# subhk/FeastKit.jl

Measured on AMD Instinct MI355X. Metric: eigenpairs/sec + max residual, 16-node contour, higher is better.
Workload: dtype f64

## Files before the change

### feastkit.jl_amd/csrc/fh_api.hip

```cpp
#include "fh_common.hpp"
#include "fh_kernels.hpp"
#include "fh_dense.hpp"
#include "fh_banded.hpp"
#include "fh_eig.hpp"
#include "fh_comm.hpp"
#include "../../include/feasthip.h"

#include <algorithm>
#include <chrono>
#include <thread>
#include <cmath>
#include <cstring>

int fh_get_buf(feasthip_ctx* h, const char* name, size_t bytes, void** out) {
    auto it = h->bufs.find(name);
    if (it != h->bufs.end() && it->second.second >= bytes) {
        *out = it->second.first;
        return 0;
    }
    if (it != h->bufs.end()) {
        hipStreamSynchronize(h->stream);
        hipFree(it->second.first);
        h->bufs.erase(it);
    }
// ... 372 lines not shown
    for (int e = 0; e < count; ++e) h->node_ids[e] = first + e;
    return 0;
}

extern "C" int feasthip_set_node_list(feasthip_handle h, int count, const int* indices) {
    if (!h) return FEASTHIP_ERROR_INTERNAL;
    if (count < 0 || (count > 0 && !indices)) { h->last_error = "feasthip_set_node_list: bad arguments"; return FEASTHIP_ERROR_FPM; }
    for (int e = 0; e < count; ++e)
        if (indices[e] < 0 || indices[e] >= (int)h->zne.size()) {
            h->last_error = "feasthip_set_node_list: index outside the contour";
            return FEASTHIP_ERROR_FPM;
        }
    h->node_ids.assign(indices, indices + count);
    h->node_first = count > 0 ? indices[0] : 0;
    h->node_count = count;
    return 0;
}

extern "C" int feasthip_set_column_mask(feasthip_handle h, int64_t m, const int* mask) {
    if (!h) return FEASTHIP_ERROR_INTERNAL;
    if (m < 0 || m > (1 << 20)) { h->last_error = "set_column_mask: m out of range"; return FEASTHIP_ERROR_M0; }
    h->col_mask.clear();
    if (mask && m > 0) h->col_mask.assign(mask, mask + m);
    return 0;
}

extern "C" int feasthip_set_solver(feasthip_handle h, int kind, double rtol, double atol, int maxit, int restart,
                                   int factor_precision, int cache_factors) {
    if (!h) return FEASTHIP_ERROR_INTERNAL;
    if (kind < 0 || kind > 4 || rtol < 0 || atol < 0 || maxit <= 0 || restart < 0 ||
        (factor_precision != 64 && factor_precision != 32)) {
        h->last_error = "feasthip_set_solver: invalid option";
        return FEASTHIP_ERROR_FPM;
    }
    h->solver = kind; h->rtol = rtol; h->atol = atol; h->maxit = maxit; h->restart = restart;
    h->factor_precision = factor_precision; h->cache_factors = cache_factors;
    return 0;
}


struct fh_op_call {
    const void* X; size_t x_stride;
    void* Y; size_t y_stride;
    const cplx* coefA; const cplx* coefB;
    const void* Bvec; size_t b_stride;
    const void* U; size_t u_stride;
    int dot_mode; cplx* partial1; cplx* partial2;
    const int* node_active;
    int nodes;
    int m = FH_MAX_LD;
    int uniform_coef = 0;
    int prec = 64;
    const cplx* colscale = nullptr;
};

static bool fh_row_kernel_ok(feasthip_ctx* h, int ld) {
    static const bool row_off = getenv("FH_SPMM_ROW") && atoi(getenv("FH_SPMM_ROW")) == 0;
    return h->kind == 2 && ld == 64 && !h->csr.is_complex && h->csr.rp8 && !row_off;
}

static int fh_apply_operator(feasthip_ctx* h, int ld, const fh_op_call& c) {
    if (h->kind == 2) {
        fh_spmm_args a;
        a.rowptr = h->csr.rowptr; a.col = h->csr.col; a.aval = h->csr.aval; a.bval = h->csr.bval;
        a.N = (int)h->csr.N; a.nodes = c.nodes;
        a.X = c.X; a.x_node_stride = c.x_stride; a.Y = c.Y; a.y_node_stride = c.y_stride;
        a.coefA = c.coefA; a.coefB = c.coefB; a.Bvec = c.Bvec; a.b_node_stride = c.b_stride;
        a.U = c.U; a.u_node_stride = c.u_stride; a.dot_mode = c.dot_mode;
        a.partial1 = c.partial1; a.partial2 = c.partial2; a.node_active = c.node_active;
        a.counters = h->profiling ? h->d_counters : nullptr; a.m = c.m; a.uniform_coef = c.uniform_coef; a.prec = c.prec;
        static const bool no_lds = !(getenv("FH_LDS_SPMM") && atoi(getenv("FH_LDS_SPMM")) != 0);
        const bool lds_kernel = h->csr.lcol && c.prec == 64 && !no_lds && c.nodes <= 64 && c.dot_mode != 6;
        a.nblk_rows = h->csr.nblk; a.blk_start = h->csr.blk_start; a.ext_ptr = h->csr.ext_ptr; a.ext_idx = h->csr.ext_idx;
        a.lcol = lds_kernel ? h->csr.lcol : nullptr;
        a.use_row_kernel = (fh_row_kernel_ok(h, ld) && !lds_kernel) ? 1 : 0;
        a.colscale = c.colscale;
        if (c.colscale && (lds_kernel || c.prec != 64 || h->csr.is_complex)) { h->last_error = "internal: column-scaled operand needs a gather kernel over a real matrix on complex128 panels"; return -1; }
        a.rp8 = h->csr.rp8; a.col8 = h->csr.col8; a.a8 = h->csr.a8; a.b8 = h->csr.b8;
        fh_prof_begin(h, "spmm");
        fh_launch_spmm(a, ld, h->csr.is_complex != 0, h->csr.b_identity != 0, fh_spmm_grid(a.N, ld), h->stream);
        fh_prof_end(h);
        if (a.use_row_kernel) return fh_spmm_row_grid(a.N);
        if (lds_kernel) return (8 / (ld / 16)) * fh_spmm_lds_slots(a.nblk_rows, ld);
        return fh_spmm_partials(a.N, ld);
    }
    fh_dense_op_args a;
    a.A = h->dense.A; a.B = h->dense.B; a.N = (int)h->dense.N; a.is_complex = h->dense.is_complex;
    a.nodes = c.nodes; a.X = (const cplx*)c.X; a.x_node_stride = c.x_stride; a.Y = (cplx*)c.Y; a.y_node_stride = c.y_stride;
    a.coefA = c.coefA; a.coefB = c.coefB; a.Bvec = (const cplx*)c.Bvec; a.b_node_stride = c.b_stride;
    a.U = (const cplx*)c.U; a.u_node_stride = c.u_stride; a.dot_mode = c.dot_mode;
    a.partial1 = c.partial1; a.partial2 = c.partial2; a.node_active = c.node_active;
    int nblk = fh_dense_op_nblk(a.N);
    fh_prof_begin(h, "dense_op");
    fh_launch_dense_op(a, ld, nblk, h->stream);
    fh_prof_end(h);
    return nblk;
}

static int fh_op_nblk(feasthip_ctx* h, int ld) {
    if (h->kind == 2) return std::max(std::max(fh_spmm_partials((int)h->csr.N, ld), ld == 64 ? fh_spmm_row_grid((int)h->csr.N) : 0),
                                      h->csr.lcol ? (8 / (ld / 16)) * fh_spmm_lds_slots(h->csr.nblk, ld) : 0);
    return fh_dense_op_nblk((int)h->dense.N);
}
static const int* fh_perm(feasthip_ctx* h) { return h->kind == 2 ? h->csr.perm : nullptr; }
static int64_t fh_N(feasthip_ctx* h) { return h->kind == 2 ? h->csr.N : h->dense.N; }
static bool fh_b_identity(feasthip_ctx* h) { return h->kind == 2 ? h->csr.b_identity != 0 : h->dense.b_identity != 0; }

static int fh_check_problem(feasthip_ctx* h, int64_t m, int wide = 0) {
    if (!h) return FEASTHIP_ERROR_INTERNAL;
    if (h->poisoned) { h->last_error = "handle poisoned by an earlier device failure: destroy it"; return FEASTHIP_ERROR_INTERNAL; }
    if (h->kind == 0) { h->last_error = "no matrix set (feasthip_set_dense / feasthip_set_csr)"; return FEASTHIP_ERROR_N; }
    if (m <= 0 || (!wide && m > FH_MAX_LD) || m > fh_N(h)) {
        h->last_error = wide ? "block width m must satisfy 1 <= m <= N" : "block width m must satisfy 1 <= m <= min(N, 64)";
        return FEASTHIP_ERROR_M0;
    }
    return 0;
}

static int fh_upload_coefs(feasthip_ctx* h, const char* name, const std::vector<cplx>& host, cplx** dev) {
    void* p = nullptr;
    int rc = fh_get_buf(h, name, host.size() * sizeof(cplx), &p);
    if (rc) return rc;
    const size_t bytes = host.size() * sizeof(cplx);
    if (h->pin && bytes <= h->pin_cap / 4) {
        const size_t need = (bytes + 63) & ~(size_t)63;
        if (h->pin_off + need > h->pin_cap) {
            FH_CHECK(hipStreamSynchronize(h->stream));
            h->pin_off = 0;
        }
        memcpy(h->pin + h->pin_off, host.data(), bytes);
// ... 118 lines not shown
    fa.atol_scale = nullptr; fa.mode = method; fa.col_mask = nullptr;
    if (h->mask_live && !h->col_mask.empty()) {
        std::vector<int> mk(ld, 1);
        for (int c = 0; c < ld && c < (int)h->col_mask.size(); ++c) mk[c] = h->col_mask[c];
        if ((rc = fh_get_buf(h, "kry_colmask", ld * sizeof(int), &p))) return rc;
        FH_CHECK(hipMemcpyAsync(p, mk.data(), ld * sizeof(int), hipMemcpyHostToDevice, h->stream));
        FH_CHECK(hipStreamSynchronize(h->stream));
        fa.col_mask = (const int*)p;
    }
    fh_vec_args va;
    memset(&va, 0, sizeof(va));
    va.N = N; va.node_stride = panel; va.R = R; va.Rhat = Rh; va.P = P; va.V = V; va.S = S; va.T = T;
    va.s = s; va.partial1 = part1; va.partial2 = part2; va.prec = prec;
    va.counters = h->profiling ? h->d_counters : nullptr;
    va.sum_acc = sum_acc; va.wnode = d_wnode; va.sum_scale = (sum_acc && prec == 32) ? r0_64 : nullptr; va.nodes = nodes;

    void* Xk = X;
    const bool shared_start = shared_src && sum_acc && method == 1 && prec == 64;
    if (shared_start) {
    } else if (prec == 64) {
        oc.prec = 64; oc.X = X; oc.x_stride = panel; oc.Y = R; oc.y_stride = panel; oc.Bvec = RHS; oc.b_stride = 0;
        oc.dot_mode = 3; oc.node_active = nullptr;
        fa.nblk = fh_apply_operator(h, ld, oc);
        res.op_calls += 1;
    } else {
        void* q;
        if ((rc = fh_get_buf(h, "kry_r64", (size_t)nodes * panel * sizeof(cplx), &q))) return rc;
        cplx* R64 = (cplx*)q;
        oc.prec = 64; oc.X = X; oc.x_stride = panel; oc.Y = R64; oc.y_stride = panel; oc.Bvec = RHS; oc.b_stride = 0;
        oc.dot_mode = 3; oc.node_active = nullptr;
        int nb = fh_apply_operator(h, ld, oc);
        res.op_calls += 1;
        fh_fin_args f0 = fa;
        f0.nblk = nb; f0.rtol = 0.0; f0.atol = 0.0; f0.mode = 0;
        fh_launch_fin_init(f0, ld, nodes, h->stream);
        FH_CHECK(hipMemcpyAsync(r0_64, s.r0norm, nl * sizeof(double), hipMemcpyDeviceToDevice, h->stream));
        cplxf* D = (cplxf*)vec(6);
        cplxf* RHS32 = (cplxf*)vec(7);
        fh_launch_narrow_scaled(R64, panel, RHS32, panel, r0_64, N, ld, nblk_vec, nodes, h->stream);
        FH_CHECK(hipMemsetAsync(D, 0, (size_t)nodes * panel * sizeof(cplxf), h->stream));
        FH_CHECK(hipMemcpyAsync(R, RHS32, (size_t)nodes * panel * sizeof(cplxf), hipMemcpyDeviceToDevice, h->stream));
        Xk = D;
        std::vector<double> hr0(nl), hinv(nl);
        FH_CHECK(hipMemcpyAsync(hr0.data(), r0_64, nl * sizeof(double), hipMemcpyDeviceToHost, h->stream));
        FH_CHECK(hipStreamSynchronize(h->stream));
        for (size_t i = 0; i < nl; ++i) hinv[i] = hr0[i] > 0 ? 1.0 / hr0[i] : 0.0;
        FH_CHECK(hipMemcpyAsync(inv_r0, hinv.data(), nl * sizeof(double), hipMemcpyHostToDevice, h->stream));
        FH_CHECK(hipStreamSynchronize(h->stream));
        fa.atol_scale = inv_r0;
    }
    va.X = Xk;
    const int vprec = prec;
    const bool lazy_off = getenv("FH_NO_LAZY_START") != nullptr;
    const bool lazy = shared_start && fused && h->kind == 2 && !h->csr.is_complex && !lazy_off && (!shared_lambda || shared_lambda_host) &&
                      !(getenv("FH_LDS_SPMM") && atoi(getenv("FH_LDS_SPMM")) != 0);
    cplx* dfs = nullptr;
    if (lazy) {
        std::vector<cplx> fs(nl, cmake(1, 0));
        if (shared_lambda_host)
            for (int e = 0; e < nodes; ++e)
                for (int c = 0; c < m; ++c) fs[(size_t)e * ld + c] = cdiv(cmake(1, 0), cmake(z[e].x - shared_lambda_host[c], z[e].y));
        if ((rc = fh_upload_coefs(h, "kry_fscale", fs, &dfs))) return rc;
        fh_vec_args vs = va;
        vs.Q = shared_src; vs.first_scale = dfs;
        fh_launch_cocg_init_lazy(vs, ld, nblk_vec, nodes, h->stream);
        fa.nblk = nblk_vec;
        fh_launch_fin_init(fa, ld, nodes, h->stream);
    } else if (shared_start) {
        fh_vec_args vs = va;
        vs.Q = shared_src; vs.lambda = shared_lambda; vs.znode = dznode;
        fh_launch_cocg_init_shared(vs, ld, nblk_vec, nodes, h->stream);
        fa.nblk = nblk_vec;
        fh_launch_fin_init(fa, ld, nodes, h->stream);
    } else if (method == 1) {
        fh_launch_cocg_init(va, ld, nblk_vec, nodes, h->stream);
        fa.nblk = nblk_vec;
        fh_launch_fin_init(fa, ld, nodes, h->stream);
    } else {
        if (prec == 32) {
            fh_launch_cocg_init(va, ld, nblk_vec, nodes, h->stream);
            fa.nblk = nblk_vec;
        }
        fa.mode = 0;
        fh_launch_fin_init(fa, ld, nodes, h->stream);
        fh_launch_copy_r(va, ld, nblk_vec, nodes, h->stream);
    }
    (void)vprec;

    oc.prec = prec; oc.Bvec = nullptr; oc.b_stride = 0; oc.x_stride = panel; oc.y_stride = panel;
    const int check_every = getenv("FH_CHECK_EVERY") ? std::max(1, atoi(getenv("FH_CHECK_EVERY"))) : 16;
    (void)d_count;
    *h->h_progress = 0ull;
    int it = 0;
    unsigned tag = 0;
    bool all_done = false;
    auto t_loop0 = std::chrono::steady_clock::now();
    auto progress = [&](unsigned& seen_tag, unsigned& seen_cnt) {
        unsigned long long w = *h->h_progress;
        seen_tag = (unsigned)(w >> 32); seen_cnt = (unsigned)(w & 0xffffffffull);
    };
    while (it < h->maxit && !all_done) {
        int chunk = std::min(check_every, h->maxit - it);
        for (int k = 0; k < chunk; ++k) {
            if (method == 0) {
                oc.X = P; oc.Y = V; oc.U = Rh; oc.u_stride = panel; oc.dot_mode = 1; oc.node_active = s.node_active;
                fa.nblk = fh_apply_operator(h, ld, oc);
                fh_prof_begin(h, "dot_finalize"); fh_launch_fin_alpha(fa, ld, nodes, h->stream); fh_prof_end(h);
                fh_prof_begin(h, "bicg_s"); fh_launch_s_update(va, ld, nblk_vec, nodes, h->stream); fh_prof_end(h);
                oc.X = S; oc.Y = T; oc.U = nullptr; oc.dot_mode = 2;
                fa.nblk = fh_apply_operator(h, ld, oc);
                fh_prof_begin(h, "dot_finalize"); fh_launch_fin_omega(fa, ld, nodes, h->stream); fh_prof_end(h);
                fh_prof_begin(h, "bicg_xr"); fh_launch_xr_update(va, ld, nblk_vec, nodes, h->stream); fh_prof_end(h);
                fa.nblk = nblk_vec;
                fh_prof_begin(h, "dot_finalize"); fh_launch_fin_rho(fa, ld, nodes, h->stream); fh_prof_end(h);
                fh_prof_begin(h, "bicg_p"); fh_launch_p_update(va, ld, nblk_vec, nodes, h->stream); fh_prof_end(h);
                res.op_calls += 2;
            } else if (fused) {
                const bool first_lazy = lazy && it + k == 0;
                oc.X = first_lazy ? (const void*)shared_src : P; oc.x_stride = first_lazy ? 0 : panel; oc.colscale = first_lazy ? dfs : nullptr;
                oc.Y = V; oc.U = nullptr; oc.dot_mode = 6; oc.node_active = s.node_active;
                oc.partial1 = sp[0]; oc.partial2 = sp[1];
                va.first_src = first_lazy ? shared_src : nullptr; va.first_scale = first_lazy ? dfs : nullptr;
                fh_fused_fin_args ff;
                ff.s = s; ff.sig = sp[0]; ff.kap = sp[1];
                ff.rho = part1; ff.rr = part2; ff.tickets = d_tickets; ff.final_check = 0;
                ff.predict_stop = (h->rtol >= 1e-3 && h->atol == 0.0) ? 1 : 0;
                ff.nblk_op = fh_apply_operator(h, ld, oc);
                ff.nblk_vec = (it + k == 0) ? fa.nblk : ((lazy && it + k == 1) ? fv1_blk * fv1_seg : fv_blk * fv_seg);
                fh_prof_begin(h, "dot_finalize"); fh_launch_fused_fin(ff, ld, nodes, h->stream); fh_prof_end(h);
                fh_prof_begin(h, "cocg_vec"); fh_launch_fused_vec(va, ld, h->stream); fh_prof_end(h);
                res.op_calls += 1;
            } else {
                oc.X = P; oc.Y = V; oc.U = nullptr; oc.dot_mode = 4; oc.node_active = s.node_active;
                fa.nblk = fh_apply_operator(h, ld, oc);
                fh_prof_begin(h, "dot_finalize"); fh_launch_fin_alpha(fa, ld, nodes, h->stream); fh_prof_end(h);
                fh_prof_begin(h, "cocg_xr"); fh_launch_cocg_update(va, ld, nblk_vec, nodes, h->stream); fh_prof_end(h);
                fa.nblk = nblk_vec;
                fh_prof_begin(h, "dot_finalize"); fh_launch_fin_rho(fa, ld, nodes, h->stream); fh_prof_end(h);
                fh_prof_begin(h, "cocg_p");
                if (sum_acc) fh_launch_cocg_p_sum(va, ld, nodes, h->stream);
                else fh_launch_cocg_p(va, ld, nblk_vec, nodes, h->stream);
                fh_prof_end(h);
                res.op_calls += 1;
            }
        }
        it += chunk;
        ++tag;
        fh_launch_publish_progress(s.node_active, nodes, h->d_progress, tag, h->stream);
        unsigned st = 0, sc = 0;
        for (unsigned spins = 1;; ++spins) {
            progress(st, sc);
            if (st >= 1 && sc == 0) { all_done = true; break; }
            if (tag < 3 || st + 3 > tag) break;
            std::this_thread::sleep_for(std::chrono::microseconds(100));
            if ((spins & 2047u) == 0) {
                const hipError_t q = hipStreamQuery(h->stream);
                if (q != hipSuccess && q != hipErrorNotReady) {
                    h->last_error = std::string("device queue failed while iterating: ") + hipGetErrorString(q);
                    h->poisoned = 1;
                    return FEASTHIP_ERROR_INTERNAL;
                }
                const double waited = std::chrono::duration<double>(std::chrono::steady_clock::now() - t_loop0).count();
                const double budget = 30.0 + 0.05 * (double)h->maxit * (1.0 + (double)N * nodes / 8.0e5);
                if (waited > budget) {
                    h->last_error = "device did not make progress on the Krylov iterations within the deadline (" + std::to_string((int)budget) + " s)";
                    fh_poison_unless_drained(h, 2.0);
                    return FEASTHIP_ERROR_INTERNAL;
                }
            }
        }
    }
    if (fused && it > 0) {
        fh_fused_fin_args ff;
        ff.s = s; ff.sig = ff.kap = nullptr; ff.rho = part1; ff.rr = part2; ff.tickets = d_tickets;
        ff.nblk_op = 0; ff.nblk_vec = (lazy && it == 1) ? fv1_blk * fv1_seg : fv_blk * fv_seg; ff.final_check = 1; ff.predict_stop = 0;
        fh_launch_fused_fin(ff, ld, nodes, h->stream);
    }
    FH_CHECK(hipStreamSynchronize(h->stream));
    if (getenv("FH_DEBUG_TIMING"))
        fprintf(stderr, "[fh_krylov] nodes=%d its queued=%d loop wall %.3f ms\n", nodes, it,
                1e3 * std::chrono::duration<double>(std::chrono::steady_clock::now() - t_loop0).count());
    if (prec == 32 && !sum_acc)
        fh_launch_widen_axpy(X, panel, (const cplxf*)Xk, panel, r0_64, N, ld, nblk_vec, nodes, h->stream);

    std::vector<int> iters(nl), status(nl), active(nl);
    std::vector<double> rnorm(nl), r0(nl);
    FH_CHECK(hipMemcpy(iters.data(), s.iters, nl * sizeof(int), hipMemcpyDeviceToHost));
    FH_CHECK(hipMemcpy(status.data(), s.status, nl * sizeof(int), hipMemcpyDeviceToHost));
    FH_CHECK(hipMemcpy(active.data(), s.active, nl * sizeof(int), hipMemcpyDeviceToHost));
    FH_CHECK(hipMemcpy(rnorm.data(), s.rnorm, nl * sizeof(double), hipMemcpyDeviceToHost));
    FH_CHECK(hipMemcpy(r0.data(), s.r0norm, nl * sizeof(double), hipMemcpyDeviceToHost));
    res.status.assign(nodes, 0);
    for (int e = 0; e < nodes; ++e) {
        int mx = 0, st = 0;
        for (int c = 0; c < m; ++c) {
            int i = e * ld + c;
            mx = std::max(mx, iters[i]);
            res.col_iters.push_back(iters[i]);
            if (active[i] || !std::isfinite(rnorm[i])) st = std::max(st, (int)FEASTHIP_ERROR_NO_CONVERGENCE);
            else if (status[i] == 8 && !(rnorm[i] <= h->atol + h->rtol * r0[i])) st = std::max(st, (int)FEASTHIP_ERROR_NO_CONVERGENCE);
            if (r0[i] > 0) res.max_rel_res = std::max(res.max_rel_res, rnorm[i] / r0[i]);
        }
        res.iters_sum += mx;
        res.node_iters.push_back(mx);
        res.max_iters = std::max(res.max_iters, mx);
        res.status[e] = st;
    }
    return 0;
}

static int fh_gmres(feasthip_ctx* h, int ld, int m, int nodes_all, const std::vector<cplx>& z, const cplx* RHS, cplx* X,
                    size_t stride, fh_solve_result& res) {
    const int N = (int)fh_N(h);
    const size_t panel = (size_t)N * ld;
    const int mr = std::max(h->restart, 2);
    int rc;
    void* p;
    res.status.assign(nodes_all, 0);
    const size_t per_node = (size_t)(mr + 2) * panel * sizeof(cplx);
    size_t budget = (size_t)48 << 30;
    {
        size_t free_b = 0, total_b = 0;
        if (hipMemGetInfo(&free_b, &total_b) == hipSuccess) {
            auto held = h->bufs.find("gm_V");
            const size_t avail = free_b / 2 + (held != h->bufs.end() ? held->second.second : 0);
            budget = std::min(budget, std::max(avail, per_node));
        }
    }
// ... 2030 lines not shown
```

### feastkit.jl_amd/csrc/fh_kernels.hpp

```cpp
#pragma once
#include "fh_common.hpp"

struct fh_spmm_args {
    const int* rowptr; const int* col; const void* aval; const void* bval;
    int N; int nodes;
    const void* X; size_t x_node_stride;
    void* Y; size_t y_node_stride;
    const cplx* coefA; const cplx* coefB;
    const void* Bvec; size_t b_node_stride;
    const void* U; size_t u_node_stride;
    int dot_mode;
    cplx* partial1; cplx* partial2;
    const int* node_active;
    unsigned long long* counters;
    int m;
    int uniform_coef;
    int prec;
    const int* rp8 = nullptr; const int* col8 = nullptr; const double* a8 = nullptr; const double* b8 = nullptr;
    int use_row_kernel = 0;
    const cplx* colscale = nullptr;
    int nblk_rows; const int* blk_start; const int* ext_ptr; const int* ext_idx; const unsigned short* lcol;
};
int fh_spmm_grid(int N, int ld);
int fh_spmm_partials(int N, int ld);
int fh_spmm_row_grid(int N);
int fh_spmm_lds_slots(int nblk_rows, int ld);
void fh_launch_spmm(const fh_spmm_args& a, int ld, bool is_complex, bool bident, int nblk, hipStream_t st);

struct fh_vec_args {
    int N;
    size_t node_stride;
    void *X, *R, *Rhat, *P, *V, *S, *T;
    const cplx* Q;
    const double* lambda;
    const cplx* znode;
    fh_krylov_scalars s;
    cplx* partial1; cplx* partial2;
    int prec;
    unsigned long long* counters;
    const cplx* first_src;
    const cplx* first_scale;
    cplx* sum_acc;
    const cplx* wnode;
    const double* sum_scale;
    int nodes;
};
struct fh_fin_args {
    fh_krylov_scalars s;
    const cplx* partial1; const cplx* partial2;
    int nblk; int m;
    double rtol, atol;
    const double* atol_scale;
    int mode;
    const int* col_mask;
};
void fh_launch_init_guess(const fh_vec_args& a, int ld, int nblk, int nodes, hipStream_t st);
void fh_launch_copy_r(const fh_vec_args& a, int ld, int nblk, int nodes, hipStream_t st);
void fh_launch_p_update(const fh_vec_args& a, int ld, int nblk, int nodes, hipStream_t st);
void fh_launch_s_update(const fh_vec_args& a, int ld, int nblk, int nodes, hipStream_t st);
void fh_launch_xr_update(const fh_vec_args& a, int ld, int nblk, int nodes, hipStream_t st);
void fh_launch_cocg_init(const fh_vec_args& a, int ld, int nblk, int nodes, hipStream_t st);
void fh_launch_cocg_init_shared(const fh_vec_args& a, int ld, int nblk, int nodes, hipStream_t st);
void fh_launch_cocg_init_lazy(const fh_vec_args& a, int ld, int nblk, int nodes, hipStream_t st);
void fh_launch_sum_finish(const cplx* src, const cplx* rho, const cplx* acc, cplx* out, int N, int ld, int real_part, hipStream_t st);
void fh_launch_cocg_update(const fh_vec_args& a, int ld, int nblk, int nodes, hipStream_t st);
void fh_launch_cocg_p(const fh_vec_args& a, int ld, int nblk, int nodes, hipStream_t st);
void fh_launch_cocg_p_sum(const fh_vec_args& a, int ld, int nodes, hipStream_t st);
struct fh_fused_fin_args {
    fh_krylov_scalars s;
    const cplx *sig, *kap;
    const cplx *rho, *rr;
    int nblk_op, nblk_vec;
    unsigned long long* tickets;
    int final_check;
    int predict_stop;
};
void fh_launch_fused_fin(const fh_fused_fin_args& a, int ld, int nodes, hipStream_t st);
void fh_fused_vec_geometry(int N, int ld, int half, int* nblk, int* nseg, int* per_thread);
void fh_launch_fused_vec(const fh_vec_args& a, int ld, hipStream_t st);
void fh_launch_fin_init(const fh_fin_args& a, int ld, int nodes, hipStream_t st);
void fh_launch_fin_alpha(const fh_fin_args& a, int ld, int nodes, hipStream_t st);
void fh_launch_fin_omega(const fh_fin_args& a, int ld, int nodes, hipStream_t st);
void fh_launch_fin_rho(const fh_fin_args& a, int ld, int nodes, hipStream_t st);
void fh_launch_count_active(const int* node_active, int nodes, int* out, hipStream_t st);
void fh_launch_publish_progress(const int* node_active, int nodes, unsigned long long* progress, unsigned tag, hipStream_t st);
void fh_launch_narrow_scaled(const cplx* src, size_t src_stride, cplxf* dst, size_t dst_stride, const double* r0norm,
                             int N, int ld, int nblk, int nodes, hipStream_t st);
void fh_launch_widen_axpy(cplx* X, size_t x_stride, const cplxf* D, size_t d_stride, const double* r0norm,
                          int N, int ld, int nblk, int nodes, hipStream_t st);

struct fh_gmres_args {
    int N; int mr;
    size_t panel;
    cplx* V; size_t v_node_stride;
    cplx* W;
    cplx* partial;
    cplx* npartial;
    cplx* H;
    cplx* hcur;
    cplx* cs; cplx* sn;
    cplx* g;
    cplx* y;
    double* inv;
    double* r0norm; double* target; double* rnorm;
    int* active; int* iters; int* status; int* kdim;
    int* node_active;
};
int fh_gm_nchunk(int k);
size_t fh_gm_partial_elems(int mr, int nblk, int nodes, int ld);
void fh_launch_gm_orthogonalize(const fh_gmres_args& a, int ld, int k, int nblk, int nodes, hipStream_t st);
void fh_launch_gm_start(const fh_gmres_args& a, int ld, int nblk_norm, int nodes, int first, double rtol, double atol, int m, hipStream_t st);
void fh_launch_gm_givens(const fh_gmres_args& a, int ld, int k, int nblk, int nodes, hipStream_t st);
void fh_launch_gm_scale_store(const fh_gmres_args& a, int ld, const cplx* src, size_t src_node_stride, int dst_index, int nblk, int nodes,
                              hipStream_t st);
void fh_launch_gm_finish_cycle(const fh_gmres_args& a, int ld, cplx* X, size_t x_node_stride, int kmax, int nblk, int nodes, hipStream_t st);

void fh_launch_to_panel(const cplx* src, int64_t lds, int N, int m, cplx* dst, int ld, hipStream_t st, const int* perm = nullptr);
void fh_launch_from_panel(const cplx* src, int ld, int N, int m, cplx* dst, int64_t ldd, hipStream_t st, const int* perm = nullptr);
void fh_launch_panel_cols(const cplx* src, int lds, int c0, int w, int N, cplx* dst, int ldd, hipStream_t st);
void fh_launch_pack_cols(const cplx* src, int lds, int c0, int w, int N, double* dst, int ldd, int real_only, hipStream_t st);
void fh_launch_to_panel_real(const double* src, int64_t lds, int N, int m, cplx* dst, int ld, hipStream_t st);
void fh_launch_accumulate(const cplx* X, size_t node_stride, const cplx* w, int nodes, int N, int ld, const cplx* extra,
                          cplx* dst, int real_part, hipStream_t st);
size_t fh_gram_work_elems(int ld);
void fh_launch_gram(const cplx* X, const cplx* Y, int N, int ld, int bilinear, cplx* work, cplx* G,
                    hipStream_t st);
int fh_vec_nblk(int N, int ld);
int fh_kry_nblk(int N, int ld, int nodes);
void fh_launch_dot_cols(const cplx* U, const cplx* V, int N, int ld, cplx* work, cplx* out, hipStream_t st);
void fh_launch_scale_cols(cplx* X, const cplx* s, int N, int ld, hipStream_t st);
void fh_launch_normalize_cols(cplx* X, const cplx* dots, int N, int ld, int M, hipStream_t st);
void fh_launch_small_matmul(const cplx* Q, const cplx* V, int N, int ld, cplx* Xout, hipStream_t st);
// ... 19 lines not shown
```

### feastkit.jl_amd/csrc/fh_sparse.hip

```cpp
#include "fh_common.hpp"
#include "fh_kernels.hpp"

#define FH_BLOCK 256
#define FH_FIN_BLOCK 1024

template <int LD>
__device__ __forceinline__ void fh_block_reduce_cols(cplx v, cplx* red, cplx* out) {
    const int t = threadIdx.x;
    red[t] = v;
    __syncthreads();
    if (t < LD) {
        cplx s = red[t];
#pragma unroll
        for (int k = 1; k < FH_BLOCK / LD; ++k) s = cadd(s, red[t + k * LD]);
        out[t] = s;
    }
    __syncthreads();
}

static inline int fh_spmm_slots(int N, int ld) {
    const int nt = ld / 16, slices = 8 / nt;
    int rows = (N + slices - 1) / slices;
    int S = (rows + 15) / 16;
    if (S > 128) S = 128;
// ... 178 lines not shown
                d2.x += cabs2(accd);
            } else if (a.dot_mode == 3) {
                d2.x += cabs2(accd);
            } else if (a.dot_mode == 4) {
                d1 = cadd(d1, cmul(to_d(xo), accd));
            } else if (a.dot_mode == 6) {
                d1 = cadd(d1, cmul(to_d(xo), accd));
                d2 = cadd(d2, cmul(accd, accd));
            }
        }
        if (a.dot_mode != 0) {
            if (a.dot_mode == 1 || a.dot_mode == 2 || a.dot_mode == 4 || a.dot_mode == 6) {
                red[t] = d1;
                __syncthreads();
                if (t < 16) {
                    cplx s = cmake(0, 0);
                    for (int k = 0; k < 16; ++k) s = cadd(s, red[t + 16 * k]);
                    a.partial1[pbase + t] = s;
                }
                __syncthreads();
            }
            if (a.dot_mode == 2 || a.dot_mode == 3 || a.dot_mode == 6) {
                red[t] = d2;
                __syncthreads();
                if (t < 16) {
                    cplx s = cmake(0, 0);
                    for (int k = 0; k < 16; ++k) s = cadd(s, red[t + 16 * k]);
                    a.partial2[pbase + t] = s;
                }
                __syncthreads();
            }
        }
    }
}

#ifndef FH_ROW_THREADS
#define FH_ROW_THREADS 1024
#endif
#ifndef FH_ROW_WAVES
#define FH_ROW_WAVES 4
#endif
#ifndef FH_ROW_BLOCKS_MAX
#define FH_ROW_BLOCKS_MAX 1
#endif
static inline int fh_spmm_row_groups(int N, int blocks_per_cu) {
    (void)N;
    return 32 * blocks_per_cu;
}

__device__ __forceinline__ double fh_uniform(double v) {
    return __hiloint2double(__builtin_amdgcn_readfirstlane(__double2hiint(v)), __builtin_amdgcn_readfirstlane(__double2loint(v)));
}

template <typename CT, bool BIDENT, bool UNIF>
__global__ __launch_bounds__(FH_ROW_THREADS, FH_ROW_WAVES) void k_spmm_row(fh_spmm_args a) {
    constexpr int LD = 64;
    __shared__ double red[FH_ROW_THREADS / 64][64][4];
    const int lane = threadIdx.x & 63;
    const int wave = __builtin_amdgcn_readfirstlane(threadIdx.x >> 6);
    constexpr int WPB = FH_ROW_THREADS / 64;
    const int S = gridDim.x >> 3;
    const int grp = blockIdx.x & 7, slot = blockIdx.x >> 3;
    const int slice_rows = (a.N + 7) / 8;
    const int row_lo = min(a.N, grp * slice_rows);
    const int row_hi = min(a.N, row_lo + slice_rows);
    const int band = S * WPB;
    typedef const double __attribute__((address_space(4))) * cdptr;
    typedef const int __attribute__((address_space(4))) * ciptr;
    const cdptr a8 = (cdptr)a.a8;
    const cdptr b8 = (cdptr)a.b8;
    const ciptr rp8 = (ciptr)a.rp8;
    const ciptr col8 = (ciptr)a.col8;
    const int prow = blockIdx.x, nprow = gridDim.x;

    for (int node = 0; node < a.nodes; ++node) {
        const size_t pbase = ((size_t)node * nprow + prow) * LD;
        if (a.node_active && a.node_active[node] == 0) {
            if (a.dot_mode != 0 && threadIdx.x < LD) {
                if (a.partial1) a.partial1[pbase + threadIdx.x] = cmake(0, 0);
                if (a.partial2) a.partial2[pbase + threadIdx.x] = cmake(0, 0);
            }
            continue;
        }
        if (a.counters && blockIdx.x == 0 && threadIdx.x == 0) {
            const int cols = a.node_active ? a.node_active[node] : a.m;
            const int passes = (a.dot_mode == 1 || a.Bvec) ? 3 : 2;
            atomicAdd(a.counters + 0, 1ull);
            atomicAdd(a.counters + 1, (unsigned long long)(cols * passes));
        }
        const CT* __restrict__ X = (const CT*)a.X + (size_t)node * a.x_node_stride;
        CT* __restrict__ Y = (CT*)a.Y + (size_t)node * a.y_node_stride;
        const CT* __restrict__ Bv = a.Bvec ? (const CT*)a.Bvec + (size_t)node * a.b_node_stride : nullptr;
        const CT* __restrict__ U = a.U ? (const CT*)a.U + (size_t)node * a.u_node_stride : nullptr;
        cplx ca = a.coefA[node * LD + lane];
        cplx cb = a.coefB[node * LD + lane];
        if (UNIF) { ca = cmake(fh_uniform(ca.x), fh_uniform(ca.y)); cb = cmake(fh_uniform(cb.x), fh_uniform(cb.y)); }
        const bool scaled = a.colscale != nullptr;
        const cplx fs = scaled ? a.colscale[node * LD + lane] : cmake(1, 0);
        double d1x = 0.0, d1y = 0.0, d2x = 0.0, d2y = 0.0;
        for (int i = row_lo + slot * WPB + wave; i < row_hi; i += band) {
            const int c0 = rp8[i], c1 = rp8[i + 1];
            double ux = 0.0, uy = 0.0, vx = 0.0, vy = 0.0;
            const CT xown = (X + (size_t)i * LD)[lane];
            for (int ch = c0; ch < c1; ++ch) {
                const ciptr cc = col8 + (size_t)ch * 8;
                const cdptr aa = a8 + (size_t)ch * 8;
                CT xs[8];
#pragma unroll
                for (int q = 0; q < 8; ++q) {
                    const int j = cc[q];
                    if (j != i) {
                        const CT* __restrict__ rowp = X + (size_t)j * LD;
                        xs[q] = rowp[lane];
                    } else {
                        xs[q] = xown;
                    }
                }
#pragma unroll
                for (int q = 0; q < 8; ++q) {
                    const cplx x = to_d(xs[q]);
                    const double av = aa[q];
                    ux += av * x.x; uy += av * x.y;
                    if (!BIDENT) {
                        const double bv = (b8 + (size_t)ch * 8)[q];
                        vx += bv * x.x; vy += bv * x.y;
                    }
                }
            }
            cplx u = cmake(ux, uy), v = cmake(vx, vy);
            if (BIDENT) v = to_d(xown);
            cplx accd = cadd(cmul(cb, v), cmul(ca, u));
            cplx xo = to_d(xown);
            if (scaled) { accd = cmul(fs, accd); xo = cmul(fs, xo); }
            if (Bv) accd = csub(to_d(fh_ld_nt((Bv + (size_t)i * LD) + lane)), accd);
            const CT acc = cvt<CT>(accd);
            fh_st_nt((Y + (size_t)i * LD) + lane, acc);
            accd = to_d(acc);
            if (a.dot_mode == 1) {
                const cplx t1 = cmulc(to_d(fh_ld_nt((U + (size_t)i * LD) + lane)), accd);
                d1x += t1.x; d1y += t1.y;
            } else if (a.dot_mode == 2) {
                const cplx t1 = cmulc(accd, xo);
                d1x += t1.x; d1y += t1.y; d2x += cabs2(accd);
            } else if (a.dot_mode == 3) {
                d2x += cabs2(accd);
            } else if (a.dot_mode == 4) {
                const cplx t1 = cmul(xo, accd);
                d1x += t1.x; d1y += t1.y;
            } else if (a.dot_mode == 6) {
                const cplx t1 = cmul(xo, accd), t2 = cmul(accd, accd);
                d1x += t1.x; d1y += t1.y; d2x += t2.x; d2y += t2.y;
            }
        }
        if (a.dot_mode != 0) {
            red[wave][lane][0] = d1x; red[wave][lane][1] = d1y; red[wave][lane][2] = d2x; red[wave][lane][3] = d2y;
            __syncthreads();
            if (threadIdx.x < LD) {
                double s0 = 0.0, s1 = 0.0, s2 = 0.0, s3 = 0.0;
#pragma unroll
                for (int w = 0; w < WPB; ++w) { s0 += red[w][threadIdx.x][0]; s1 += red[w][threadIdx.x][1]; s2 += red[w][threadIdx.x][2]; s3 += red[w][threadIdx.x][3]; }
                if (a.partial1) a.partial1[pbase + threadIdx.x] = cmake(s0, s1);
                if (a.partial2) a.partial2[pbase + threadIdx.x] = cmake(s2, s3);
            }
            __syncthreads();
        }
    }
}

#define FH_LDS_SLOTS (FH_SPMM_R + FH_SPMM_EXT)
#define FH_LDS_RPG (FH_SPMM_R / 16)
#define FH_SEL8(arr, s) ((s) == 0 ? arr[0] : (s) == 1 ? arr[1] : (s) == 2 ? arr[2] : (s) == 3 ? arr[3] : (s) == 4 ? arr[4] : (s) == 5 ? arr[5] : (s) == 6 ? arr[6] : arr[7])
static_assert(FH_LDS_RPG == 8, "FH_SEL8 assumes eight rows per lane group");
template <typename VT, int LD, bool BIDENT>
__global__ __launch_bounds__(FH_BLOCK, 2) void k_spmm_lds(fh_spmm_args a) {
    typedef cplx CT;
    constexpr int NT = LD / 16;
    constexpr int SLICES = 8 / NT;
    extern __shared__ cplx lds_x[];
    __shared__ cplx red[FH_BLOCK];
    __shared__ int s_list[64];
    __shared__ int s_cnt;
    const int t = threadIdx.x;
    const int lane = t & 63, wave = t >> 6;
    const int g = lane >> 4, l16 = lane & 15;
    const int S = gridDim.x >> 3;
    const int grp = blockIdx.x & 7, slot = blockIdx.x >> 3;
    const int ct = grp % NT, slice = grp / NT;
    const int per = (a.nblk_rows + SLICES - 1) / SLICES;
    const int b_lo = min(a.nblk_rows, slice * per), b_hi = min(a.nblk_rows, b_lo + per);
    const int c = ct * 16 + l16;
    const VT* __restrict__ aval = (const VT*)a.aval;
    const VT* __restrict__ bval = (const VT*)a.bval;
    const int* __restrict__ rowptr = a.rowptr;
    const int* __restrict__ colidx = a.col;
    const unsigned short* __restrict__ lcol = a.lcol;
    const int prow = slice * S + slot;
    const int nprow = SLICES * S;

    if (t == 0) {
        int n = 0;
        for (int node = 0; node < a.nodes && n < 64; ++node)
            if (!a.node_active || a.node_active[node] != 0) s_list[n++] = node;
        s_cnt = n;
    }
    if (a.dot_mode != 0 && t < 16) {
        for (int node = 0; node < a.nodes; ++node) {
            const size_t pb = ((size_t)node * nprow + prow) * LD + ct * 16;
            if (a.partial1) a.partial1[pb + t] = cmake(0, 0);
            if (a.partial2) a.partial2[pb + t] = cmake(0, 0);
        }
    }
    __syncthreads();
    const int cnt_nodes = s_cnt;
    if (a.counters && blockIdx.x == 0 && t == 0) {
        unsigned long long cols = 0;
        for (int q = 0; q < cnt_nodes; ++q) cols += (unsigned long long)(a.node_active ? a.node_active[s_list[q]] : a.m);
        atomicAdd(a.counters + 0, (unsigned long long)cnt_nodes);
// ... 164 lines not shown
        hipFuncSetAttribute((const void*)k_spmm_lds<VT, LD, true>, hipFuncAttributeMaxDynamicSharedMemorySize, (int)dyn);
        hipFuncSetAttribute((const void*)k_spmm_lds<VT, LD, false>, hipFuncAttributeMaxDynamicSharedMemorySize, (int)dyn);
        attr_done = true;
    }
    dim3 grid(8 * fh_spmm_lds_slots(a.nblk_rows, LD)), block(FH_BLOCK);
    if (bident) hipLaunchKernelGGL((k_spmm_lds<VT, LD, true>), grid, block, dyn, st, a);
    else hipLaunchKernelGGL((k_spmm_lds<VT, LD, false>), grid, block, dyn, st, a);
}

template <typename CT, typename VT, int LD>
static void launch_spmm_ld(const fh_spmm_args& a, bool bident, int nblk, hipStream_t st) {
    dim3 grid(nblk), block(FH_BLOCK);
    if constexpr (sizeof(CT) == sizeof(cplx) && sizeof(VT) == sizeof(double)) {
        if (a.colscale) {
            if (bident) hipLaunchKernelGGL((k_spmm<CT, VT, LD, true, true>), grid, block, 0, st, a);
            else hipLaunchKernelGGL((k_spmm<CT, VT, LD, false, true>), grid, block, 0, st, a);
            return;
        }
    }
    if (bident)
        hipLaunchKernelGGL((k_spmm<CT, VT, LD, true>), grid, block, 0, st, a);
    else
        hipLaunchKernelGGL((k_spmm<CT, VT, LD, false>), grid, block, 0, st, a);
}
template <typename CT>
static void launch_spmm_ct(const fh_spmm_args& a, int ld, bool is_complex, bool bident, int nblk, hipStream_t st) {
    if (is_complex) {
        if (ld == 16) launch_spmm_ld<CT, cplx, 16>(a, bident, nblk, st);
        else if (ld == 32) launch_spmm_ld<CT, cplx, 32>(a, bident, nblk, st);
        else launch_spmm_ld<CT, cplx, 64>(a, bident, nblk, st);
    } else {
        if (ld == 16) launch_spmm_ld<CT, double, 16>(a, bident, nblk, st);
        else if (ld == 32) launch_spmm_ld<CT, double, 32>(a, bident, nblk, st);
        else launch_spmm_ld<CT, double, 64>(a, bident, nblk, st);
    }
}
int fh_spmm_row_grid(int N) {
    static int per_cu = 0;
    if (!per_cu) {
        int n = 0;
        if (hipOccupancyMaxActiveBlocksPerMultiprocessor(&n, k_spmm_row<cplx, false, true>, FH_ROW_THREADS, 0) != hipSuccess || n < 1) n = 1;
        per_cu = n > FH_ROW_BLOCKS_MAX ? FH_ROW_BLOCKS_MAX : n;
    }
    int S = fh_spmm_row_groups(N, per_cu);
    const int slice_rows = (N + 7) / 8, wpb = FH_ROW_THREADS / 64;
    const int need = (slice_rows + wpb - 1) / wpb;
    if (S > need) S = need < 1 ? 1 : need;
    return 8 * S;
}

void fh_launch_spmm(const fh_spmm_args& a, int ld, bool is_complex, bool bident, int nblk, hipStream_t st) {
    if (a.use_row_kernel) {
        dim3 grid(fh_spmm_row_grid(a.N)), block(FH_ROW_THREADS);
#define FH_ROW_LAUNCH(CT_, BI_) \
        do { if (a.uniform_coef) hipLaunchKernelGGL((k_spmm_row<CT_, BI_, true>), grid, block, 0, st, a); \
             else hipLaunchKernelGGL((k_spmm_row<CT_, BI_, false>), grid, block, 0, st, a); } while (0)
        if (a.prec == 32) { if (bident) FH_ROW_LAUNCH(cplxf, true); else FH_ROW_LAUNCH(cplxf, false); }
        else { if (bident) FH_ROW_LAUNCH(cplx, true); else FH_ROW_LAUNCH(cplx, false); }
#undef FH_ROW_LAUNCH
        return;
    }
    if (a.prec == 64 && a.lcol) {
        if (is_complex) {
            if (ld == 16) launch_spmm_lds<cplx, 16>(a, bident, st);
            else if (ld == 32) launch_spmm_lds<cplx, 32>(a, bident, st);
            else launch_spmm_lds<cplx, 64>(a, bident, st);
        } else {
            if (ld == 16) launch_spmm_lds<double, 16>(a, bident, st);
            else if (ld == 32) launch_spmm_lds<double, 32>(a, bident, st);
            else launch_spmm_lds<double, 64>(a, bident, st);
        }
        return;
    }
    if (a.prec == 32) launch_spmm_ct<cplxf>(a, ld, is_complex, bident, nblk, st);
    else launch_spmm_ct<cplx>(a, ld, is_complex, bident, nblk, st);
}

template <typename CT, int LD>
__global__ __launch_bounds__(FH_BLOCK) void k_init_guess(fh_vec_args a) {
    const int node = blockIdx.y;
    const size_t total = (size_t)a.N * LD;
    const int c = threadIdx.x % LD;
    cplx* X = (cplx*)a.X + (size_t)node * a.node_stride;
    cplx f = cmake(0, 0);
    if (a.lambda) {
        cplx z = a.znode[node];
        f = cdiv(cmake(1, 0), cmake(z.x - a.lambda[c], z.y));
    }
    for (size_t e = (size_t)blockIdx.x * FH_BLOCK + threadIdx.x; e < total; e += (size_t)gridDim.x * FH_BLOCK)
        X[e] = a.lambda ? cmul(a.Q[e], f) : cmake(0, 0);
}

template <typename CT, int LD>
__global__ __launch_bounds__(FH_BLOCK) void k_copy_r(fh_vec_args a) {
    const int node = blockIdx.y;
    const size_t total = (size_t)a.N * LD;
    const CT* R = (const CT*)a.R + (size_t)node * a.node_stride;
    CT* Rh = (CT*)a.Rhat + (size_t)node * a.node_stride;
    CT* P = (CT*)a.P + (size_t)node * a.node_stride;
    for (size_t e = (size_t)blockIdx.x * FH_BLOCK + threadIdx.x; e < total; e += (size_t)gridDim.x * FH_BLOCK) {
        CT r = R[e];
        Rh[e] = r;
        P[e] = r;
    }
}

template <typename CT, int LD>
__global__ __launch_bounds__(FH_BLOCK) void k_p_update(fh_vec_args a) {
    const int node = blockIdx.y;
    if (a.s.node_active[node] == 0) return;
    const size_t total = (size_t)a.N * LD;
    const int c = threadIdx.x % LD;
    if (!a.s.active[node * LD + c]) return;
    const CT beta = cvt<CT>(a.s.beta[node * LD + c]), omega = cvt<CT>(a.s.omega[node * LD + c]);
    const CT* R = (const CT*)a.R + (size_t)node * a.node_stride;
    const CT* V = (const CT*)a.V + (size_t)node * a.node_stride;
    CT* P = (CT*)a.P + (size_t)node * a.node_stride;
    for (size_t e = (size_t)blockIdx.x * FH_BLOCK + threadIdx.x; e < total; e += (size_t)gridDim.x * FH_BLOCK) {
        CT t = csub(P[e], cmul(omega, V[e]));
        P[e] = cadd(R[e], cmul(beta, t));
    }
}

template <typename CT, int LD>
__global__ __launch_bounds__(FH_BLOCK) void k_s_update(fh_vec_args a) {
    const int node = blockIdx.y;
    if (a.s.node_active[node] == 0) return;
    const size_t total = (size_t)a.N * LD;
// ... 804 lines not shown
```

Baseline: 301.2.

## Fuse COCG vector update with recomputed SpMM to skip storing A*p

The fused COCG path normally writes the operator product V = A*P, then a separate vector kernel reads it back to update R, P and the solution sum. The new mode runs the SpMM with dots only and no store, and a new row kernel recomputes A*P per row while applying the residual, direction and accumulation updates. P and V ping-pong as the input and output direction buffers, and the kernel processes nodes in groups of up to four. This removes a full panel write and read per iteration but computes the sparse product twice, so it trades memory traffic for extra gathers and FLOPs.

Measured after the change: 293.5 (median of 2 runs). 0.974x the previous value.

```diff
diff --git a/feastkit.jl_amd/csrc/fh_api.hip b/feastkit.jl_amd/csrc/fh_api.hip
--- a/feastkit.jl_amd/csrc/fh_api.hip
+++ b/feastkit.jl_amd/csrc/fh_api.hip
@@ -448,6 +448,7 @@
     int uniform_coef = 0;
     int prec = 64;
     const cplx* colscale = nullptr;
+    int no_store = 0;
 };
 
 static bool fh_row_kernel_ok(feasthip_ctx* h, int ld) {
@@ -472,6 +473,8 @@
         a.use_row_kernel = (fh_row_kernel_ok(h, ld) && !lds_kernel) ? 1 : 0;
         a.colscale = c.colscale;
         if (c.colscale && (lds_kernel || c.prec != 64 || h->csr.is_complex)) { h->last_error = "internal: column-scaled operand needs a gather kernel over a real matrix on complex128 panels"; return -1; }
+        a.no_store = c.no_store;
+        if (c.no_store && (!a.use_row_kernel || c.prec != 64 || c.dot_mode != 6 || !c.uniform_coef || c.Bvec || c.colscale)) { h->last_error = "internal: dots-only operator product needs the row kernel, fused-COCG dots and complex128 panels"; return -1; }
         a.rp8 = h->csr.rp8; a.col8 = h->csr.col8; a.a8 = h->csr.a8; a.b8 = h->csr.b8;
         fh_prof_begin(h, "spmm");
         fh_launch_spmm(a, ld, h->csr.is_complex != 0, h->csr.b_identity != 0, fh_spmm_grid(a.N, ld), h->stream);
@@ -696,6 +699,9 @@
     va.X = Xk;
     const int vprec = prec;
     const bool lazy_off = getenv("FH_NO_LAZY_START") != nullptr;
+    const bool cocg_row = fused && sum_acc && prec == 64 && ld == 64 && fh_row_kernel_ok(h, ld) &&
+                          !(getenv("FH_COCG_ROW") && atoi(getenv("FH_COCG_ROW")) == 0);
+    const int cocg_group = getenv("FH_COCG_GROUP") ? std::max(1, std::min(4, atoi(getenv("FH_COCG_GROUP")))) : 4;
     const bool lazy = shared_start && fused && h->kind == 2 && !h->csr.is_complex && !lazy_off && (!shared_lambda || shared_lambda_host) &&
                       !(getenv("FH_LDS_SPMM") && atoi(getenv("FH_LDS_SPMM")) != 0);
     cplx* dfs = nullptr;
@@ -732,6 +738,15 @@
     (void)vprec;
 
     oc.prec = prec; oc.Bvec = nullptr; oc.b_stride = 0; oc.x_stride = panel; oc.y_stride = panel;
+    int vec_rows = fa.nblk;
+    fh_cocg_row_args ra;
+    memset(&ra, 0, sizeof(ra));
+    if (cocg_row) {
+        ra.N = N; ra.nodes = nodes; ra.node_stride = panel;
+        ra.rp8 = h->csr.rp8; ra.col8 = h->csr.col8; ra.a8 = h->csr.a8; ra.b8 = h->csr.b8;
+        ra.coefA = dca; ra.coefB = dcb; ra.R = (cplx*)R; ra.sum_acc = sum_acc; ra.wnode = d_wnode;
+        ra.s = s; ra.partial1 = part1; ra.partial2 = part2; ra.counters = va.counters;
+    }
     const int check_every = getenv("FH_CHECK_EVERY") ? std::max(1, atoi(getenv("FH_CHECK_EVERY"))) : 16;
     (void)d_count;
     *h->h_progress = 0ull;
@@ -761,8 +776,11 @@
                 res.op_calls += 2;
             } else if (fused) {
                 const bool first_lazy = lazy && it + k == 0;
-                oc.X = first_lazy ? (const void*)shared_src : P; oc.x_stride = first_lazy ? 0 : panel; oc.colscale = first_lazy ? dfs : nullptr;
-                oc.Y = V; oc.U = nullptr; oc.dot_mode = 6; oc.node_active = s.node_active;
+                const bool gu = cocg_row && !first_lazy;
+                const bool odd = gu && ((it + k - (lazy ? 1 : 0)) & 1);
+                void* Pin = odd ? V : P;
+                oc.X = first_lazy ? (const void*)shared_src : Pin; oc.x_stride = first_lazy ? 0 : panel; oc.colscale = first_lazy ? dfs : nullptr;
+                oc.Y = gu ? nullptr : V; oc.no_store = gu ? 1 : 0; oc.U = nullptr; oc.dot_mode = 6; oc.node_active = s.node_active;
                 oc.partial1 = sp[0]; oc.partial2 = sp[1];
                 va.first_src = first_lazy ? shared_src : nullptr; va.first_scale = first_lazy ? dfs : nullptr;
                 fh_fused_fin_args ff;
@@ -770,9 +788,17 @@
                 ff.rho = part1; ff.rr = part2; ff.tickets = d_tickets; ff.final_check = 0;
                 ff.predict_stop = (h->rtol >= 1e-3 && h->atol == 0.0) ? 1 : 0;
                 ff.nblk_op = fh_apply_operator(h, ld, oc);
-                ff.nblk_vec = (it + k == 0) ? fa.nblk : ((lazy && it + k == 1) ? fv1_blk * fv1_seg : fv_blk * fv_seg);
+                ff.nblk_vec = vec_rows;
                 fh_prof_begin(h, "dot_finalize"); fh_launch_fused_fin(ff, ld, nodes, h->stream); fh_prof_end(h);
-                fh_prof_begin(h, "cocg_vec"); fh_launch_fused_vec(va, ld, h->stream); fh_prof_end(h);
+                fh_prof_begin(h, "cocg_vec");
+                if (gu) {
+                    ra.Pin = (const cplx*)Pin; ra.Pout = (cplx*)(odd ? P : V);
+                    vec_rows = fh_launch_cocg_row(ra, h->csr.b_identity != 0, cocg_group, h->stream);
+                } else {
+                    fh_launch_fused_vec(va, ld, h->stream);
+                    vec_rows = first_lazy ? fv1_blk * fv1_seg : fv_blk * fv_seg;
+                }
+                fh_prof_end(h);
                 res.op_calls += 1;
             } else {
                 oc.X = P; oc.Y = V; oc.U = nullptr; oc.dot_mode = 4; oc.node_active = s.node_active;
@@ -817,7 +843,7 @@
     if (fused && it > 0) {
         fh_fused_fin_args ff;
         ff.s = s; ff.sig = ff.kap = nullptr; ff.rho = part1; ff.rr = part2; ff.tickets = d_tickets;
-        ff.nblk_op = 0; ff.nblk_vec = (lazy && it == 1) ? fv1_blk * fv1_seg : fv_blk * fv_seg; ff.final_check = 1; ff.predict_stop = 0;
+        ff.nblk_op = 0; ff.nblk_vec = vec_rows; ff.final_check = 1; ff.predict_stop = 0;
         fh_launch_fused_fin(ff, ld, nodes, h->stream);
     }
     FH_CHECK(hipStreamSynchronize(h->stream));
diff --git a/feastkit.jl_amd/csrc/fh_kernels.hpp b/feastkit.jl_amd/csrc/fh_kernels.hpp
--- a/feastkit.jl_amd/csrc/fh_kernels.hpp
+++ b/feastkit.jl_amd/csrc/fh_kernels.hpp
@@ -18,6 +18,7 @@
     int prec;
     const int* rp8 = nullptr; const int* col8 = nullptr; const double* a8 = nullptr; const double* b8 = nullptr;
     int use_row_kernel = 0;
+    int no_store = 0;
     const cplx* colscale = nullptr;
     int nblk_rows; const int* blk_start; const int* ext_ptr; const int* ext_idx; const unsigned short* lcol;
 };
@@ -78,6 +79,18 @@
 void fh_launch_fused_fin(const fh_fused_fin_args& a, int ld, int nodes, hipStream_t st);
 void fh_fused_vec_geometry(int N, int ld, int half, int* nblk, int* nseg, int* per_thread);
 void fh_launch_fused_vec(const fh_vec_args& a, int ld, hipStream_t st);
+struct fh_cocg_row_args {
+    int N; int nodes;
+    size_t node_stride;
+    const int* rp8; const int* col8; const double* a8; const double* b8;
+    const cplx* coefA; const cplx* coefB;
+    const cplx* Pin; cplx* Pout; cplx* R;
+    cplx* sum_acc; const cplx* wnode;
+    fh_krylov_scalars s;
+    cplx* partial1; cplx* partial2;
+    unsigned long long* counters;
+};
+int fh_launch_cocg_row(const fh_cocg_row_args& a, bool bident, int group, hipStream_t st);
 void fh_launch_fin_init(const fh_fin_args& a, int ld, int nodes, hipStream_t st);
 void fh_launch_fin_alpha(const fh_fin_args& a, int ld, int nodes, hipStream_t st);
 void fh_launch_fin_omega(const fh_fin_args& a, int ld, int nodes, hipStream_t st);
diff --git a/feastkit.jl_amd/csrc/fh_sparse.hip b/feastkit.jl_amd/csrc/fh_sparse.hip
--- a/feastkit.jl_amd/csrc/fh_sparse.hip
+++ b/feastkit.jl_amd/csrc/fh_sparse.hip
@@ -254,7 +254,47 @@
     return __hiloint2double(__builtin_amdgcn_readfirstlane(__double2hiint(v)), __builtin_amdgcn_readfirstlane(__double2loint(v)));
 }
 
-template <typename CT, bool BIDENT, bool UNIF>
+typedef const double __attribute__((address_space(4))) * fh_cdptr;
+typedef const int __attribute__((address_space(4))) * fh_ciptr;
+
+template <typename CT, bool BIDENT>
+__device__ __forceinline__ cplx fh_row_apply(fh_ciptr rp8, fh_ciptr col8, fh_cdptr a8, fh_cdptr b8, const CT* __restrict__ X, int i,
+                                             int lane, cplx ca, cplx cb, CT& xown) {
+    constexpr int LD = 64;
+    const int c0 = rp8[i], c1 = rp8[i + 1];
+    double ux = 0.0, uy = 0.0, vx = 0.0, vy = 0.0;
+    xown = (X + (size_t)i * LD)[lane];
+    for (int ch = c0; ch < c1; ++ch) {
+        const fh_ciptr cc = col8 + (size_t)ch * 8;
+        const fh_cdptr aa = a8 + (size_t)ch * 8;
+        CT xs[8];
+#pragma unroll
+        for (int q = 0; q < 8; ++q) {
+            const int j = cc[q];
+            if (j != i) {
+                const CT* __restrict__ rowp = X + (size_t)j * LD;
+                xs[q] = rowp[lane];
+            } else {
+                xs[q] = xown;
+            }
+        }
+#pragma unroll
+        for (int q = 0; q < 8; ++q) {
+            const cplx x = to_d(xs[q]);
+            const double av = aa[q];
+            ux += av * x.x; uy += av * x.y;
+            if (!BIDENT) {
+                const double bv = (b8 + (size_t)ch * 8)[q];
+                vx += bv * x.x; vy += bv * x.y;
+            }
+        }
+    }
+    cplx u = cmake(ux, uy), v = cmake(vx, vy);
+    if (BIDENT) v = to_d(xown);
+    return cadd(cmul(cb, v), cmul(ca, u));
+}
+
+template <typename CT, bool BIDENT, bool UNIF, bool NOSTORE = false>
 __global__ __launch_bounds__(FH_ROW_THREADS, FH_ROW_WAVES) void k_spmm_row(fh_spmm_args a) {
     constexpr int LD = 64;
     __shared__ double red[FH_ROW_THREADS / 64][64][4];
@@ -267,12 +307,10 @@
     const int row_lo = min(a.N, grp * slice_rows);
     const int row_hi = min(a.N, row_lo + slice_rows);
     const int band = S * WPB;
-    typedef const double __attribute__((address_space(4))) * cdptr;
-    typedef const int __attribute__((address_space(4))) * ciptr;
-    const cdptr a8 = (cdptr)a.a8;
-    const cdptr b8 = (cdptr)a.b8;
-    const ciptr rp8 = (ciptr)a.rp8;
-    const ciptr col8 = (ciptr)a.col8;
+    const fh_cdptr a8 = (fh_cdptr)a.a8;
+    const fh_cdptr b8 = (fh_cdptr)a.b8;
+    const fh_ciptr rp8 = (fh_ciptr)a.rp8;
+    const fh_ciptr col8 = (fh_ciptr)a.col8;
     const int prow = blockIdx.x, nprow = gridDim.x;
 
     for (int node = 0; node < a.nodes; ++node) {
@@ -286,7 +324,7 @@
         }
         if (a.counters && blockIdx.x == 0 && threadIdx.x == 0) {
             const int cols = a.node_active ? a.node_active[node] : a.m;
-            const int passes = (a.dot_mode == 1 || a.Bvec) ? 3 : 2;
+            const int passes = NOSTORE ? 1 : (a.dot_mode == 1 || a.Bvec) ? 3 : 2;
             atomicAdd(a.counters + 0, 1ull);
             atomicAdd(a.counters + 1, (unsigned long long)(cols * passes));
         }
@@ -301,42 +339,13 @@
         const cplx fs = scaled ? a.colscale[node * LD + lane] : cmake(1, 0);
         double d1x = 0.0, d1y = 0.0, d2x = 0.0, d2y = 0.0;
         for (int i = row_lo + slot * WPB + wave; i < row_hi; i += band) {
-            const int c0 = rp8[i], c1 = rp8[i + 1];
-            double ux = 0.0, uy = 0.0, vx = 0.0, vy = 0.0;
-            const CT xown = (X + (size_t)i * LD)[lane];
-            for (int ch = c0; ch < c1; ++ch) {
-                const ciptr cc = col8 + (size_t)ch * 8;
-                const cdptr aa = a8 + (size_t)ch * 8;
-                CT xs[8];
-#pragma unroll
-                for (int q = 0; q < 8; ++q) {
-                    const int j = cc[q];
-                    if (j != i) {
-                        const CT* __restrict__ rowp = X + (size_t)j * LD;
-                        xs[q] = rowp[lane];
-                    } else {
-                        xs[q] = xown;
-                    }
-                }
-#pragma unroll
-                for (int q = 0; q < 8; ++q) {
-                    const cplx x = to_d(xs[q]);
-                    const double av = aa[q];
-                    ux += av * x.x; uy += av * x.y;
-                    if (!BIDENT) {
-                        const double bv = (b8 + (size_t)ch * 8)[q];
-                        vx += bv * x.x; vy += bv * x.y;
-                    }
-                }
-            }
-            cplx u = cmake(ux, uy), v = cmake(vx, vy);
-            if (BIDENT) v = to_d(xown);
-            cplx accd = cadd(cmul(cb, v), cmul(ca, u));
+            CT xown;
+            cplx accd = fh_row_apply<CT, BIDENT>(rp8, col8, a8, b8, X, i, lane, ca, cb, xown);
             cplx xo = to_d(xown);
             if (scaled) { accd = cmul(fs, accd); xo = cmul(fs, xo); }
             if (Bv) accd = csub(to_d(fh_ld_nt((Bv + (size_t)i * LD) + lane)), accd);
             const CT acc = cvt<CT>(accd);
-            fh_st_nt((Y + (size_t)i * LD) + lane, acc);
+            if (!NOSTORE) fh_st_nt((Y + (size_t)i * LD) + lane, acc);
             accd = to_d(acc);
             if (a.dot_mode == 1) {
                 const cplx t1 = cmulc(to_d(fh_ld_nt((U + (size_t)i * LD) + lane)), accd);
@@ -365,6 +374,109 @@
                 if (a.partial2) a.partial2[pbase + threadIdx.x] = cmake(s2, s3);
             }
             __syncthreads();
+        }
+    }
+}
+
+template <bool BIDENT, int G>
+__global__ __launch_bounds__(FH_ROW_THREADS, FH_ROW_WAVES) void k_cocg_row(fh_cocg_row_args a) {
+    constexpr int LD = 64;
+    constexpr int WPB = FH_ROW_THREADS / 64;
+    __shared__ double red[WPB][64][3];
+    __shared__ cplx s_alpha[G][LD], s_beta[G][LD];
+    const int lane = threadIdx.x & 63;
+    const int wave = __builtin_amdgcn_readfirstlane(threadIdx.x >> 6);
+    const int S = gridDim.x >> 3;
+    const int grp = blockIdx.x & 7, slot = blockIdx.x >> 3;
+    const int slice_rows = (a.N + 7) / 8;
+    const int row_lo = min(a.N, grp * slice_rows);
+    const int row_hi = min(a.N, row_lo + slice_rows);
+    const int band = S * WPB;
+    const fh_cdptr a8 = (fh_cdptr)a.a8;
+    const fh_cdptr b8 = (fh_cdptr)a.b8;
+    const fh_ciptr rp8 = (fh_ciptr)a.rp8;
+    const fh_ciptr col8 = (fh_ciptr)a.col8;
+    const fh_cdptr cA = (fh_cdptr)a.coefA;
+    const fh_cdptr cB = (fh_cdptr)a.coefB;
+    const fh_cdptr wn = (fh_cdptr)a.wnode;
+    const fh_ciptr nacc = (fh_ciptr)a.s.node_accum;
+    const fh_ciptr nact = (fh_ciptr)a.s.node_active;
+    const int prow = blockIdx.x, nprow = gridDim.x;
+
+    for (int g0 = 0; g0 < a.nodes; g0 += G) {
+        const int gn = min(G, a.nodes - g0);
+        unsigned stepm = 0, actm = 0;
+        bool group_any = false;
+#pragma unroll
+        for (int k = 0; k < G; ++k) {
+            const int n = g0 + k;
+            if (k < gn && nacc[n] != 0) {
+                group_any = true;
+                const int ci = n * LD + lane;
+                if (a.s.accum[ci]) stepm |= 1u << k;
+                if (a.s.active[ci]) actm |= 1u << k;
+                if (threadIdx.x < LD) { s_alpha[k][lane] = a.s.alpha[ci]; s_beta[k][lane] = a.s.beta[ci]; }
+                if (a.counters && blockIdx.x == 0 && threadIdx.x == 0) {
+                    atomicAdd(a.counters + 2, (unsigned long long)nacc[n]);
+                    atomicAdd(a.counters + 3, (unsigned long long)nact[n]);
+                }
+            } else if (k < gn && threadIdx.x < LD) {
+                const size_t o = ((size_t)n * nprow + prow) * LD + lane;
+                a.partial1[o] = cmake(0, 0);
+                a.partial2[o] = cmake(0, 0);
+            }
+        }
+        if (!group_any) continue;
+        if (a.counters && blockIdx.x == 0 && threadIdx.x < LD && stepm) atomicAdd(a.counters + 4, 1ull);
+        __syncthreads();
+        double d[G][3];
+#pragma unroll
+        for (int k = 0; k < G; ++k) d[k][0] = d[k][1] = d[k][2] = 0.0;
+        for (int i = row_lo + slot * WPB + wave; i < row_hi; i += band) {
+            const size_t e = (size_t)i * LD + lane;
+            cplx acc = cmake(0, 0);
+#pragma unroll
+            for (int k = 0; k < G; ++k) {
+                const int n = g0 + k;
+                if (k < gn && nacc[n] != 0) {
+                    const size_t off = (size_t)n * a.node_stride;
+                    const bool step = (stepm >> k) & 1u, act = (actm >> k) & 1u;
+                    cplx rv = cmake(0, 0), q = cmake(0, 0), pv;
+                    if (act) rv = fh_ld_nt(a.R + off + e);
+                    if (nact[n] != 0) {
+                        const cplx ca = cmake(cA[2 * n * LD], cA[2 * n * LD + 1]), cb = cmake(cB[2 * n * LD], cB[2 * n * LD + 1]);
+                        q = fh_row_apply<cplx, BIDENT>(rp8, col8, a8, b8, a.Pin + off, i, lane, ca, cb, pv);
+                    } else {
+                        pv = a.Pin[off + e];
+                    }
+                    const cplx alpha = s_alpha[k][lane];
+                    if (step) cfma(acc, cmul(cmake(wn[2 * n], wn[2 * n + 1]), alpha), pv);
+                    if (act) {
+                        const cplx rn = csub(rv, cmul(alpha, q));
+                        fh_st_nt(a.R + off + e, rn);
+                        fh_st_nt(a.Pout + off + e, cadd(rn, cmul(s_beta[k][lane], pv)));
+                        d[k][0] += rn.x * rn.x - rn.y * rn.y; d[k][1] += 2.0 * rn.x * rn.y; d[k][2] += cabs2(rn);
+                    }
+                }
+            }
+            if (stepm) a.sum_acc[e] = cadd(a.sum_acc[e], acc);
+        }
+#pragma unroll
+        for (int k = 0; k < G; ++k) {
+            const int n = g0 + k;
+            if (k < gn && nacc[n] != 0) {
+                red[wave][lane][0] = d[k][0]; red[wave][lane][1] = d[k][1]; red[wave][lane][2] = d[k][2];
+                __syncthreads();
+                if (threadIdx.x < LD) {
+                    double s0 = 0.0, s1 = 0.0, s2 = 0.0;
+#pragma unroll
+                    for (int w = 0; w < WPB; ++w) { s0 += red[w][threadIdx.x][0]; s1 += red[w][threadIdx.x][1]; s2 += red[w][threadIdx.x][2]; }
+                    const size_t o = ((size_t)n * nprow + prow) * LD + threadIdx.x;
+                    a.partial1[o] = cmake(s0, s1);
+                    a.partial2[o] = cmake(s2, 0.0);
+                }
+                __syncthreads();
+            }
         }
     }
 }
@@ -635,6 +747,11 @@
 void fh_launch_spmm(const fh_spmm_args& a, int ld, bool is_complex, bool bident, int nblk, hipStream_t st) {
     if (a.use_row_kernel) {
         dim3 grid(fh_spmm_row_grid(a.N)), block(FH_ROW_THREADS);
+        if (a.no_store) {
+            if (bident) hipLaunchKernelGGL((k_spmm_row<cplx, true, true, true>), grid, block, 0, st, a);
+            else hipLaunchKernelGGL((k_spmm_row<cplx, false, true, true>), grid, block, 0, st, a);
+            return;
+        }
 #define FH_ROW_LAUNCH(CT_, BI_) \
         do { if (a.uniform_coef) hipLaunchKernelGGL((k_spmm_row<CT_, BI_, true>), grid, block, 0, st, a); \
              else hipLaunchKernelGGL((k_spmm_row<CT_, BI_, false>), grid, block, 0, st, a); } while (0)
@@ -657,6 +774,19 @@
     }
     if (a.prec == 32) launch_spmm_ct<cplxf>(a, ld, is_complex, bident, nblk, st);
     else launch_spmm_ct<cplx>(a, ld, is_complex, bident, nblk, st);
+}
+
+int fh_launch_cocg_row(const fh_cocg_row_args& a, bool bident, int group, hipStream_t st) {
+    const int nblk = fh_spmm_row_grid(a.N);
+    const dim3 grid(nblk), block(FH_ROW_THREADS);
+#define FH_COCG_ROW_LAUNCH(G_) \
+    do { if (bident) hipLaunchKernelGGL((k_cocg_row<true, G_>), grid, block, 0, st, a); \
+         else hipLaunchKernelGGL((k_cocg_row<false, G_>), grid, block, 0, st, a); } while (0)
+    if (group <= 1) FH_COCG_ROW_LAUNCH(1);
+    else if (group == 2) FH_COCG_ROW_LAUNCH(2);
+    else FH_COCG_ROW_LAUNCH(4);
+#undef FH_COCG_ROW_LAUNCH
+    return nblk;
 }
 
 template <typename CT, int LD>
```
